# ztaylor797/APMBackend

Measured on AMD Instinct MI355X. Metric: log-lines/sec z-scored (whole node), higher is better.
Workload: dtype fp64

## Files before the change

### apmbackend_amd/csrc/kernels/devjoin.hip

```cpp
#include "kernel_api.h"

#include <rocprim/rocprim.hpp>

#include <chrono>
#include <climits>
#include <cstdlib>
#include <cstddef>
#include <cstring>
#include <vector>

#include "devjoin_api.h"
#include "devjoin_dev.h"
#include "devscan.h"
#include "prim.h"
#include "textout.h"

namespace apm {
using namespace dj;

namespace {

constexpr int TB = 256;

__device__ __forceinline__ uint32_t grid_n(uint32_t n) { return (n + TB - 1) / TB; }
// ... 2254 lines not shown

int apm_dj_take_marks(double* t, const char** names, int cap) {
  const int k = std::min(g_mark_k, cap);
  for (int i = 0; i < k; ++i) { t[i] = g_mark_t[i]; names[i] = g_mark_n[i]; }
  g_mark_k = 0;
  return k;
}

static int dj_sort_keys(PrimScratch& sc, const uint64_t* key, uint64_t* key_sorted, const uint32_t* val,
                        uint32_t* val_sorted, size_t n, hipStream_t s) {
  return prim_sort_pairs(sc, key, key_sorted, val, val_sorted, n, s);
}
static int dj_scan_counts(PrimScratch& sc, const uint32_t* cnt, uint32_t* pos, size_t n, hipStream_t s) {
  return prim_exclusive_scan(sc, cnt, pos, 0u, n, rocprim::plus<uint32_t>(), s);
}
static int dj_scan_lens(PrimScratch& sc, const U4* lens, U4* offs, size_t n, hipStream_t s) {
  return prim_exclusive_scan(sc, lens, offs, U4{0, 0, 0, 0}, n, U4Plus(), s);
}
static int dj_scan_bucket_max(PrimScratch& sc, const int64_t* bucket, int64_t* bmax, size_t n, hipStream_t s) {
  return prim_inclusive_scan(sc, bucket, bmax, n, rocprim::maximum<int64_t>(), s);
}

size_t apm_dj_tmp_bytes(uint32_t max_ev, uint32_t max_out) {
  PrimScratch q;
  const size_t n = std::max<size_t>(max_ev, 1) + 1;
  dj_sort_keys(q, nullptr, nullptr, nullptr, nullptr, n, 0);
  dj_scan_counts(q, nullptr, nullptr, n, 0);
  dj_scan_lens(q, nullptr, nullptr, (size_t)max_out + 1, 0);
  dj_scan_bucket_max(q, nullptr, nullptr, (size_t)max_out + 1, 0);
  return q.need + 4096;
}

int apm_dj_select_host(DJArgs* a, const uint32_t* d_n_ev, uint32_t max_ev, hipStream_t s) {
  HIP_OK(hipMemsetAsync(a->n_host, 0, sizeof(SelCount), s));
  if (max_ev == 0) return 0;
  uint32_t* list = reinterpret_cast<uint32_t*>(a->sel_pos);
  uint32_t* list_n = list + max_ev;
  HIP_OK(hipMemsetAsync(list_n, 0, 8, s));
  const dim3 grid((max_ev + TB - 1) / TB);
  hipLaunchKernelGGL(k_host_flags, grid, dim3(TB), 0, s, a->ev, d_n_ev, a->bytes, a->host_flag, a->sel_val, a->aud,
                     a->n_host, max_ev, list, list_n);
  dj_check(s, "k_host_flags");
  hipLaunchKernelGGL(k_host_flags_bytes, grid, dim3(TB), 0, s, a->ev, a->bytes, a->chunk_file, a->file_fkey,
                     a->host_flag, a->sel_val, a->aud, max_ev, list, list_n);
  dj_check(s, "k_host_flags_bytes");
  uint64_t* total = a->sel_pos + (max_ev + DS_TILE - 1) / DS_TILE + 1;
  if (ds_scan_apply<uint64_t>(SelValF{a->sel_val},
                              SelScatterG{a->ev, a->host_flag, total, a->host_ev, a->host_ev_idx, a->mh_idx,
                                          a->walk_idx, a->n_host},
                              d_n_ev, max_ev, a->sel_pos, total, s) != 0)
    return -1;
  dj_check(s, "k_ds_scan (host selection)");
  return 0;
}

static int apm_dj_audit(DJArgs* a, bool filled, hipStream_t s) {
  if (a->n_files && !filled) HIP_OK(hipMemsetAsync(a->gout.carry, 0, (size_t)a->n_files * sizeof(AudCarry), s));
  const uint32_t N = a->gin.n_autr + a->n_mh;
  if (N) {
    hipLaunchKernelGGL(k_aud_keys, dim3((N + TB - 1) / TB), dim3(TB), 0, s, *a);
    dj_check(s, "k_aud_keys");
    PrimScratch sc(a->tmp, a->tmp_bytes);
    if (dj_sort_keys(sc, a->aud_key, a->aud_key_sorted, a->aud_ord, a->aud_ord_sorted, N, s) != 0) return -1;
    dj_check(s, "rocprim_radix_sort_pairs");
    hipLaunchKernelGGL(k_aud_autr, dim3((N + TB - 1) / TB), dim3(TB), 0, s, *a);
    dj_check(s, "k_aud_autr");
  }
  if (a->n_walk || a->gin.n_txt) {
    if (a->n_files && !filled) HIP_OK(hipMemsetAsync(a->file_first_chunk, 0xff, (size_t)a->n_files * 4, s));
    const uint32_t lanes = std::max(a->n_chunks + 1, a->n_walk + 1);
    hipLaunchKernelGGL(k_aud_chunks, dim3((lanes + TB - 1) / TB), dim3(TB), 0, s, *a);
// ... 319 lines not shown
```

### apmbackend_amd/csrc/kernels/devjoin_api.h

```cpp
#pragma once
#include <vector>
#include <hip/hip_runtime.h>
#include <stdint.h>

#include "../apm_types.h"
#include "devjoin_types.h"

namespace apm {

constexpr int SOAP_SEGS = 16;
constexpr uint32_t DJ_OVF_CAP = 1u << 16;

enum : uint32_t {
  DJ_WRITE_OK = 0,
  DJ_WRITE_TXT = 1,
  DJ_WRITE_TOO_BIG = 2,
  DJ_WRITE_RING_FULL = 3,
};

__host__ __device__ inline uint64_t ring_place(uint64_t head, uint64_t bytes, uint64_t cap) {
  return ((head & (cap - 1)) + bytes > cap) ? (head + cap - 1) & ~(cap - 1) : head;
}

struct DJOverflow {
  uint32_t ev, sub;
  uint32_t pad[14];
  TxDev t;
};

struct AudGen {
  AudCarry* carry;
  AutrEnt* autr;
  AudItem* items;
  char* txt;
  uint32_t n_autr, n_items, n_txt;
  uint32_t cap_autr, cap_items, cap_txt;
};

struct SelCount {
  uint32_t host;
  uint32_t mh;
  uint32_t walk;
  uint32_t aud_bytes;
};

struct DJArgs {
  const Event* ev;
  uint32_t n_ev;
  const uint8_t* bytes;
  const uint32_t* chunk_file;
  const uint8_t* chunk_kind;
  uint32_t n_chunks;
  const int32_t* chunk_next;
  const uint8_t* chunk_first;
  const int32_t* file_server;
  const uint64_t* file_skey;
  const uint64_t* file_fkey;
  const HostOp* hops;
  uint32_t n_hops;
  const uint8_t* hbuf;
  double now;
  uint64_t batch_no;
  double rec_ttl, acct_ttl, need_ttl;
  uint8_t* host_flag;
  uint64_t* sel_val;
  uint64_t* sel_pos;
  Event* host_ev;
  uint32_t* host_ev_idx;
  uint32_t* mh_idx;
  uint32_t* walk_idx;
  SelCount* n_host;
  uint32_t n_mh, n_walk;
  uint32_t n_files;
  AudF* aud;
  AudGen gin, gout;
  uint64_t* aud_key;
  uint64_t* aud_key_sorted;
// ... 144 lines not shown
```

### apmbackend_amd/csrc/kernels/kernel_api.h

```cpp
#pragma once
#include <hip/hip_runtime.h>
#include <stdint.h>

#include "../apm_types.h"
#include "common.h"

namespace apm {

struct StatsState {
  int32_t* counts;
  int32_t* cells;
  int32_t* spill_n;
  int32_t* spill_series;
  int32_t* spill_val;
  uint8_t* active;
  int32_t cap;
  int32_t spill_cap;
  int32_t S;
  int32_t nslot = NSLOT_MIN;
  unsigned long long* spill_drop = nullptr;
  int32_t* nan_until = nullptr;
  int32_t* ord_list = nullptr;
  int32_t* ord_n = nullptr;
  uint32_t* ord_done = nullptr;
// ... 41 lines not shown
  int32_t rs_lo, rs_n, rs_parts;
  int32_t rs_mfma;
  double* rs_part;
  int32_t* rs_cnt;
};

constexpr int ROLLUP_ACC = 6;
constexpr int ROLLUP_OUT = 15;
constexpr int CTX_FIELDS = 18;
struct RollupArgs {
  const WinStat* win;
  const int32_t* series_server;
  const ZOut* z[MAX_LAGS];
  int32_t n_lags;
  int32_t n_series;
  int32_t n_servers;
  int64_t edge_ts;
  double tpm_div;
  const double* ctx;
  unsigned long long* acc;
  double* out;
};

struct CopySeg {
  void* dst;
  const void* src;
  size_t bytes;
};
struct CopySegs {
  CopySeg seg[8];
  int32_t n = 0;
  void add(void* d, const void* s, size_t b) {
    if (b) seg[n++] = CopySeg{d, s, b};
  }
};

struct ExportArgs {
  static constexpr int kMax = 8;
  void* src[kMax];
  void* dst[kMax];
  uint64_t reset_val[kMax];
  uint8_t bytes[kMax];
  uint8_t reset[kMax];
  int32_t n;
  void add(void* s, void* d, int nb, bool rst = false, uint64_t rv = 0) {
    src[n] = s; dst[n] = d; bytes[n] = (uint8_t)nb; reset[n] = rst ? 1 : 0; reset_val[n] = rv; ++n;
  }
};

struct FormatArgs {
  const int32_t* perm;
  const WinStat* win;
  const ZOut* z[MAX_LAGS];
  const int4* series_names;
  const char* names;
  int64_t edge_ts;
  int32_t n;
  int32_t n_lags;
  int32_t lag_order[MAX_LAGS];
  int32_t lag_value[MAX_LAGS];
  int32_t want_st, want_fs;
  int32_t fs_copy;
  uint32_t stage_hint;
  int32_t ts_copy_len;
  char ts_copy[32];
  int32_t ts_wire_len;
// ... 222 lines not shown
```

### apmbackend_amd/csrc/kernels/stats.hip

```cpp
#include "kernel_api.h"

#include "prim.h"
#include "spill.h"
#include "winsort.h"

#include <algorithm>
#include <cstdlib>

namespace apm {

constexpr int WS_WAVES = 4;
constexpr int WS_TILE = 1024;
constexpr int BIG_TILE = 16384;

__global__ void k_bucket_append(const TxRec* __restrict__ tx, uint32_t lo, uint32_t hi, StatsState st,
                                int64_t min_live_bucket) {
  const uint32_t i = lo + blockIdx.x * blockDim.x + threadIdx.x;
  if (i >= hi) return;
  const TxRec r = tx[i];
  if (r.series < 0 || r.series >= st.S) return;
  st.active[r.series] = 1;
  const int64_t b = r.end_ms / 10000;
  if (b < min_live_bucket) return;
  if (st.nan_until && b <= (int64_t)st.nan_until[r.series]) {
// ... 709 lines not shown
  for (; i < n; i += stride) dst[i] = src[i];
  if (t0 < tail) tdst[t0] = tsrc[t0];
}

}

__global__ void k_ck_lens(const int32_t* __restrict__ counts, const int32_t* __restrict__ slots, int k, int32_t n,
                          int32_t S, int32_t cap, uint32_t* __restrict__ lens) {
  const uint64_t t = (uint64_t)blockIdx.x * blockDim.x + threadIdx.x;
  const uint64_t N = (uint64_t)k * n;
  if (t > N) return;
  if (t == N) { lens[N] = 0; return; }
  const int i = (int)(t / (uint64_t)n), s = (int)(t % (uint64_t)n);
  const int32_t c = counts[(size_t)slots[i] * S + s];
  lens[t] = (uint32_t)(c < cap ? (c > 0 ? c : 0) : cap);
}

__global__ void k_ck_pack(const int32_t* __restrict__ cells, const int32_t* __restrict__ slots, int k, int32_t n,
                          int32_t S, int32_t cap, const uint32_t* __restrict__ lens, const uint32_t* __restrict__ offs,
                          int32_t* __restrict__ packed) {
  const uint64_t t = (uint64_t)blockIdx.x * blockDim.x + threadIdx.x;
  if (t >= (uint64_t)k * n) return;
  const int i = (int)(t / (uint64_t)n), s = (int)(t % (uint64_t)n);
  const int32_t* src = cells + ((size_t)slots[i] * S + s) * cap;
  int32_t* dst = packed + offs[t];
  for (uint32_t j = 0; j < lens[t]; ++j) dst[j] = src[j];
}

__global__ void k_copy_segs(apm::CopySegs c) {
  const apm::CopySeg& g = c.seg[blockIdx.y];
  if (blockIdx.y >= (unsigned)c.n) return;
  const size_t stride = (size_t)gridDim.x * blockDim.x;
  const size_t t = (size_t)blockIdx.x * blockDim.x + threadIdx.x;
  const uintptr_t al = (uintptr_t)g.dst | (uintptr_t)g.src;
  if ((al & 15) == 0) {
    const size_t n16 = g.bytes / 16;
    for (size_t i = t; i < n16; i += stride) reinterpret_cast<uint4*>(g.dst)[i] = reinterpret_cast<const uint4*>(g.src)[i];
    for (size_t i = n16 * 16 + t; i < g.bytes; i += stride) ((uint8_t*)g.dst)[i] = ((const uint8_t*)g.src)[i];
  } else if ((al & 3) == 0) {
    const size_t n4 = g.bytes / 4;
    for (size_t i = t; i < n4; i += stride) reinterpret_cast<uint32_t*>(g.dst)[i] = reinterpret_cast<const uint32_t*>(g.src)[i];
    for (size_t i = n4 * 4 + t; i < g.bytes; i += stride) ((uint8_t*)g.dst)[i] = ((const uint8_t*)g.src)[i];
  } else {
    for (size_t i = t; i < g.bytes; i += stride) ((uint8_t*)g.dst)[i] = ((const uint8_t*)g.src)[i];
  }
}

struct F64x8 {
  double v[8];
};
__global__ void k_set_f64(double* __restrict__ dst, F64x8 v, int n) {
  if ((int)threadIdx.x < n) dst[threadIdx.x] = v.v[threadIdx.x];
}

extern "C" {

using namespace apm;

void apm_copy(void* dst, const void* src, size_t bytes, hipStream_t stream) {
  apm_copy_capped(dst, src, bytes, 1024, stream);
}

void apm_copy_capped(void* dst, const void* src, size_t bytes, uint32_t max_blocks, hipStream_t stream) {
  if (bytes == 0) return;
  const uintptr_t a = (uintptr_t)dst | (uintptr_t)src;
  auto launch = [&](auto* d, const auto* s, size_t w) {
// ... 147 lines not shown
```

### apmbackend_amd/csrc/runtime/devjoin.cpp

```cpp
#include "devjoin.h"

#include <algorithm>
#include <chrono>
#include <climits>
#include <cstddef>
#include <cstdlib>
#include <cstring>
#include <stdexcept>

#include "../kernels/common.h"
#include "binio.h"
#include "d2h.h"
#include "../kernels/devjoin_dev.h"
#include "../kernels/kernel_api.h"
#include "join_util.h"
#include "jsutil.h"

namespace apm {

using namespace jstr;

namespace {
double clock_ms() {
  return std::chrono::duration<double, std::milli>(std::chrono::steady_clock::now().time_since_epoch()).count();
// ... 6 lines not shown
  op.line = e.line;
  op.server = server;
  op.op = JOP_NONE;
  return op;
}

uint64_t pow2_at_least(uint64_t v) {
  uint64_t p = 1;
  while (p < v) p <<= 1;
  return p;
}
}

DeviceJoin::DeviceJoin(const DevJoinConfig& cfg, Dictionary* dict, const std::vector<FileInfo>* files,
                       const std::vector<std::string>* servers)
    : cfg_(cfg), dict_(dict), files_(files), servers_(servers) {
  cfg_.ring_bytes = pow2_at_least(std::max<uint64_t>(cfg_.ring_bytes, 1ull << 24));
  cfg_.arena_cap = (uint32_t)pow2_at_least(std::max<uint32_t>(cfg_.arena_cap, 1024));
  HIP_OK(hipSetDevice(cfg_.device));
  {
    int lo = 0, hi = 0;
    HIP_OK(hipDeviceGetStreamPriorityRange(&lo, &hi));
    const char* pe = std::getenv("APM_JOIN_PRIO");
    HIP_OK(hipStreamCreateWithPriority(&stream_, hipStreamNonBlocking, pe && pe[0] == '0' ? lo : hi));
    res_.adopt(stream_);
  }
  const uint32_t E = std::max<uint32_t>(cfg_.max_events, 1024);
  out_cap_ = 2 * E + (1u << 16);
  for (int k = 0; k < 2; ++k) {
    Slot& s = sl_[k];
    s.d_bytes = (uint8_t*)res_.dmalloc_on(stream_, cfg_.max_batch_bytes + 256);
    s.d_events = (Event*)res_.dmalloc_on(stream_, (size_t)E * sizeof(Event));
    s.host_flag = (uint8_t*)res_.dmalloc_on(stream_, E + 64);
    s.d_host_ev = (Event*)res_.dmalloc_on(stream_, (size_t)E * sizeof(Event));
    s.d_host_idx = (uint32_t*)res_.dmalloc_on(stream_, (size_t)E * 4);
    s.d_mh_idx = (uint32_t*)res_.dmalloc_on(stream_, (size_t)E * 4);
    s.d_walk_idx = (uint32_t*)res_.dmalloc_on(stream_, (size_t)E * 4);
    s.d_aud = (AudF*)res_.dmalloc_on(stream_, (size_t)E * sizeof(AudF));
    s.d_n_host = (SelCount*)res_.dmalloc_on(stream_, 64);
    res_.pin(s.h_host_ev, (size_t)E * sizeof(Event));
    res_.pin(s.h_host_idx, (size_t)E * 4);
    res_.pin(s.h_n_host, 64);
    std::memset(s.h_n_host, 0, 64);
    s.d_chunk_next = (int32_t*)res_.dmalloc_on(stream_, ((size_t)cfg_.max_chunks + 2) * 4);
    s.d_chunk_first = (uint8_t*)res_.dmalloc_on(stream_, (size_t)cfg_.max_chunks + 2);
    res_.pin(s.h_chunk_next, ((size_t)cfg_.max_chunks + 2) * 4);
    res_.pin(s.h_chunk_first, (size_t)cfg_.max_chunks + 2);
    s.d_tx = (TxRec*)res_.dmalloc_on(stream_, (size_t)out_cap_ * sizeof(TxRec));
    s.d_tx_raw = (int32_t*)res_.dmalloc_on(stream_, (size_t)out_cap_ * 4);
    s.d_tx_gid = (int64_t*)res_.dmalloc_on(stream_, (size_t)out_cap_ * 8);
    s.free_ev = res_.new_event();
  }
  table_cap_ = 1u << cfg_.table_bits;
  init_table_cap_ = table_cap_;
  init_arena_cap_ = cfg_.arena_cap;
  d_table_ = (KeyState*)res_.dmalloc_on(stream_, (size_t)table_cap_ * sizeof(KeyState));
  d_reg_ = (RegSlot*)res_.dmalloc_on(stream_, ((size_t)1 << cfg_.reg_bits) * sizeof(RegSlot));
  miss_cap_ = E;
  d_miss_ = (RegMiss*)res_.dmalloc_on(stream_, (size_t)miss_cap_ * sizeof(RegMiss));
  res_.pin(h_miss_, (size_t)miss_cap_ * sizeof(RegMiss));
  d_arena_ = (NeedEnt*)res_.dmalloc_on(stream_, (size_t)cfg_.arena_cap * sizeof(NeedEnt));
  d_exp_lo_ = (uint64_t*)res_.dmalloc_on(stream_, 8 * 4096);
  d_exp_hi_ = (uint64_t*)res_.dmalloc_on(stream_, 8 * 4096);
  res_.pin(h_exp_, 2 * 8 * 4096);
  soap_cap_ = 1u << 16;
  d_soap_ = (SoapState*)res_.dmalloc_on(stream_, (size_t)soap_cap_ * sizeof(SoapState));
  if (E >= (1u << 21)) throw std::runtime_error("device join: gpu.maxLinesPerBatch must be below 2^21");
  d_sel_val_ = (uint64_t*)res_.dmalloc_on(stream_, ((size_t)E + 64) * 8);
  d_sel_pos_ = (uint64_t*)res_.dmalloc_on(stream_, ((size_t)E + 64) * 8);
  d_walk_lo_ = (uint32_t*)res_.dmalloc_on(stream_, ((size_t)cfg_.max_chunks + 2) * 4);
  d_file_first_ = (int32_t*)res_.dmalloc_on(stream_, (size_t)soap_cap_ * 4);
  for (AudGen& g : aud_gen_) {
    g.carry = (AudCarry*)res_.dmalloc_on(stream_, (size_t)soap_cap_ * sizeof(AudCarry));
    aud_reserve(g, 4096, 16384, 1u << 20);
  }
  d_file_server_ = (int32_t*)res_.dmalloc_on(stream_, (size_t)soap_cap_ * 4);
// ... 77 lines not shown
DeviceJoin::~DeviceJoin() {
  hipStreamSynchronize(stream_);
  res_.release_all();
}

void DeviceJoin::sync_file_keys() {
  const size_t n = files_->size();
  if (n <= h_file_fkey_.size()) return;
  if (n > soap_cap_) throw std::runtime_error("device join: too many files");
  const size_t lo = h_file_fkey_.size();
  if (lo == 0) HIP_OK(hipStreamSynchronize(stream_));
  for (size_t i = lo; i < n; ++i) {
    const FileInfo& f = (*files_)[i];
    const std::string& srv = (*servers_)[f.server];
    h_file_skey_.push_back(dj::server_key_of(srv.data(), srv.size()));
    h_file_fkey_.push_back(dj::file_key_of(f.path.data(), f.path.size()));
  }
  HIP_OK(hipMemcpy(d_file_skey_ + lo, h_file_skey_.data() + lo, (n - lo) * 8, hipMemcpyHostToDevice));
  HIP_OK(hipMemcpy(d_file_fkey_ + lo, h_file_fkey_.data() + lo, (n - lo) * 8, hipMemcpyHostToDevice));
}

void DeviceJoin::select_host(int k, const uint32_t* d_n_ev, uint32_t max_ev, hipStream_t ps) {
  Slot& s = sl_[k];
  sync_file_keys();
  DJArgs a{};
  a.ev = s.d_events;
  a.bytes = s.d_bytes;
  a.host_flag = s.host_flag;
  a.chunk_file = s.d_chunk_file;
  a.file_fkey = d_file_fkey_;
  a.aud = s.d_aud;
  a.sel_val = d_sel_val_;
  a.sel_pos = d_sel_pos_;
  a.host_ev = s.d_host_ev;
  a.host_ev_idx = s.d_host_idx;
  a.mh_idx = s.d_mh_idx;
  a.walk_idx = s.d_walk_idx;
  a.n_host = s.d_n_host;
  a.tmp = d_sel_tmp_;
  a.tmp_bytes = sel_tmp_bytes_;
  if (apm_dj_select_host(&a, d_n_ev, std::min<uint32_t>(max_ev, cfg_.max_events), ps) != 0)
    throw std::runtime_error("device join: scan scratch too small");
  HIP_OK(hipMemcpyAsync(s.h_n_host, s.d_n_host, sizeof(SelCount), hipMemcpyDeviceToHost, ps));
  s.spec = std::min<uint32_t>(cfg_.max_events, last_host_ + last_host_ / 4 + 256);
  HIP_OK(hipMemcpyAsync(s.h_host_ev, s.d_host_ev, (size_t)s.spec * sizeof(Event), hipMemcpyDeviceToHost, ps));
  HIP_OK(hipMemcpyAsync(s.h_host_idx, s.d_host_idx, (size_t)s.spec * 4, hipMemcpyDeviceToHost, ps));
}

void DeviceJoin::set_chunks(int k, const std::vector<int32_t>& chunk_file, const uint32_t* d_chunk_file,
                            const uint8_t* d_chunk_kind, hipStream_t ps) {
  Slot& s = sl_[k];
  const uint32_t n = (uint32_t)chunk_file.size();
  std::unordered_map<int32_t, int32_t> last;
  for (uint32_t c = 0; c < n; ++c) {
    s.h_chunk_next[c] = -1;
    auto it = last.find(chunk_file[c]);
    if (it == last.end()) {
      s.h_chunk_first[c] = 1;
    } else {
      s.h_chunk_first[c] = 0;
      s.h_chunk_next[it->second] = (int32_t)c;
    }
    last[chunk_file[c]] = (int32_t)c;
  }
  if (n) {
    HIP_OK(hipMemcpyAsync(s.d_chunk_next, s.h_chunk_next, (size_t)n * 4, hipMemcpyHostToDevice, ps));
    HIP_OK(hipMemcpyAsync(s.d_chunk_first, s.h_chunk_first, n, hipMemcpyHostToDevice, ps));
  }
  s.d_chunk_file = d_chunk_file;
  s.d_chunk_kind = d_chunk_kind;
  s.n_chunks = n;
  s.chunk_file = chunk_file;
}

void DeviceJoin::finish_select(int k, hipStream_t ps) {
  Slot& s = sl_[k];
  const uint32_t n = s.h_n_host->host;
  if (n > s.spec) {
    HIP_OK(hipMemcpyAsync(s.h_host_ev + s.spec, s.d_host_ev + s.spec, (size_t)(n - s.spec) * sizeof(Event),
                          hipMemcpyDeviceToHost, ps));
    HIP_OK(hipMemcpyAsync(s.h_host_idx + s.spec, s.d_host_idx + s.spec, (size_t)(n - s.spec) * 4,
                          hipMemcpyDeviceToHost, ps));
    HIP_OK(hipStreamSynchronize(ps));
  }
  last_host_ = n;
}

void DeviceJoin::host_prepass(int k, const uint8_t* hb, uint32_t n_host, const ParallelFor& parallel,
                              std::vector<HostOp>& hops_out, std::string& hbuf_out) {
  Slot& s = sl_[k];
  hops_out.clear();
  hbuf_out.clear();
  std::unordered_map<int32_t, int> task_of;
  int nt = 0;
  int32_t last_file = -1;
  int last_t = -1;
  for (uint32_t i = 0; i < n_host; ++i) {
    const int32_t file = s.chunk_file[s.h_host_ev[i].chunk];
    if (file == last_file) {
      tasks_[last_t].idx.push_back(i);
      continue;
    }
    auto it = task_of.find(file);
    int t;
    if (it == task_of.end()) {
      t = nt++;
      task_of.emplace(file, t);
      if ((int)tasks_.size() < nt) tasks_.emplace_back();
      PrepassTask& T = tasks_[t];
      T.file = file;
      T.idx.clear(); T.hops.clear(); T.hbuf.clear();
      T.audit_errors = T.invalid_acct = T.pm_host = 0;
    } else {
      t = it->second;
    }
    last_file = file;
    last_t = t;
    tasks_[t].idx.push_back(i);
// ... 483 lines not shown
    HIP_OK(hipEventSynchronize(live_ev_));
    keys_live_ = *h_live_;
    live_pending_ = false;
  }
  if ((keys_live_ + keys_since_rebuild_ + n_ev) * 2 > table_cap_) {
    if (table_rebuilds_ > 0 && async_rebuild_fits(n_ev)) {
      rebuild_table_async(now);
      return ensure_rest(n_ev, bytes);
    }
    rebuild_table(now, table_cap_);
    uint64_t cap = table_cap_;
    while ((keys_live_ + n_ev) * 2 > cap) cap *= 2;
    if (cap >= (1ull << 31)) throw std::runtime_error("device join: key table beyond 2^31 slots");
    if (cap != table_cap_) rebuild_table(now, (uint32_t)cap);
  }
  ensure_rest(n_ev, bytes);
}

void DeviceJoin::ensure_rest(uint32_t n_ev, uint64_t bytes) {
  {
    const uint64_t low = regions_.empty() ? arena_head_ : regions_.front().lo;
    const uint64_t used = arena_head_ - low;
    uint64_t cap = cfg_.arena_cap;
    while (cap - used < n_ev) cap *= 2;
    if (cap >= (1ull << 31)) throw std::runtime_error("device join: need arena beyond 2^31 entries");
    if (cap != cfg_.arena_cap) grow_arena((uint32_t)cap, low);
  }
  const uint64_t need = 2ull * n_ev + bytes / LBLK_N + 64;
  if (pool_avail(false) < need && pool_avail(true) < need) grow_pool(need);
}

void DeviceJoin::prepass_ahead(int k, const uint8_t* hb, const ParallelFor& parallel) {
  if (ahead_k_ >= 0) throw std::runtime_error("device join: a pre-pass is already ahead");
  host_prepass(k, hb, sl_[k].h_n_host->host, parallel, hops_ahead_, hbuf_ahead_);
  ahead_k_ = k;
}

void DeviceJoin::run(int k, const uint8_t* hb, uint32_t n_ev, uint64_t n_bytes, double now, uint64_t batch_no,
                     bool want_tx, bool want_db, DevJoinBatch& out, const ParallelFor& parallel,
                     const std::function<void()>* meanwhile) {
  Slot& s = sl_[k];
  hipStream_t st = stream_;
  if (n_ev > cfg_.max_events) throw std::runtime_error("device join: more events than maxLinesPerBatch");
  events_ += n_ev;
  phase_t[0] = clock_ms();
  if (ahead_k_ == k) {
    std::swap(hops_, hops_ahead_);
    std::swap(hbuf_, hbuf_ahead_);
    ahead_k_ = -1;
  } else {
    if (ahead_k_ >= 0) throw std::runtime_error("device join: pre-pass ahead for another slot");
    host_prepass(k, hb, s.h_n_host->host, parallel, hops_, hbuf_);
  }
  phase_t[1] = clock_ms();
  spans.clear();
  double sp = phase_t[1];
  auto span = [&](const char* name) { const double t = clock_ms(); spans.push_back({name, {sp, t}}); sp = t; };
  res_.reserve(h_hops_, hops_.size(), hops_.size() * 2 + 65536, true);
  res_.reserve(h_hbuf_, hbuf_.size(), hbuf_.size() * 2 + (4 << 20), true);
  span("u.hostgrow");
  if (hops_.size() > d_hops_cap_) {
    d_hops_cap_ = hops_.size() * 2 + 65536;
    d_hops_ = (HostOp*)res_.dmalloc_raw(d_hops_cap_ * sizeof(HostOp));
  }
  if (hbuf_.size() > d_hbuf_cap_) {
    d_hbuf_cap_ = hbuf_.size() * 2 + (4 << 20);
    d_hbuf_ = (uint8_t*)res_.dmalloc_raw(d_hbuf_cap_);
  }
  span("u.devgrow");
  if (!hops_.empty()) {
    std::memcpy(h_hops_, hops_.data(), hops_.size() * sizeof(HostOp));
    span("u.hops.memcpy");
    apm_copy(d_hops_, h_hops_.d, hops_.size() * sizeof(HostOp), st);
    span("u.hops.h2d");
  }
  if (!hbuf_.empty()) {
    std::memcpy(h_hbuf_, hbuf_.data(), hbuf_.size());
    span("u.hbuf.memcpy");
    apm_copy(d_hbuf_, h_hbuf_.d, hbuf_.size(), st);
    span("u.hbuf.h2d");
  }
  sync_file_keys();
  if (files_->size() > files_uploaded_) {
    if (files_->size() > soap_cap_) throw std::runtime_error("device join: too many files");
    std::vector<int32_t> fs(files_->size() - files_uploaded_);
// ... 704 lines not shown
```

### apmbackend_amd/csrc/runtime/devjoin.h

```cpp
#pragma once
#include <hip/hip_runtime.h>

#include <atomic>
#include <cstdint>
#include <deque>
#include <functional>
#include <mutex>
#include <string>
#include <unordered_map>
#include <vector>

#include "../apm_types.h"
#include "../kernels/devjoin_api.h"
#include "hipres.h"
#include "join.h"

namespace apm {

struct DevJoinConfig {
  uint32_t max_events = 1u << 20;
  uint64_t max_batch_bytes = 64ull << 20;
  uint32_t max_chunks = 4096;
  int table_bits = 21;
  int reg_bits = 20;
  uint32_t max_raw = 1u << 20;
  uint32_t arena_cap = 1u << 20;
  uint32_t pool_blocks = 0;
  uint64_t ring_bytes = 4ull << 30;
  double record_ttl_ms = 120000, acct_ttl_ms = 120000, need_ttl_ms = 30000;
  TzTable tz{};
  int device = 0;
};

struct DevJoinBatch {
  int slot = 0;
  uint32_t n_out = 0, n_stats = 0, n_db = 0, n_dropped = 0;
  std::vector<std::pair<uint32_t, int64_t>> cands;
  std::vector<std::pair<uint32_t, int32_t>> unresolved;
  std::string text_tx, text_db;
  uint64_t ring_base = 0;
  int64_t max_bucket = INT64_MIN;
  TxRec* d_tx = nullptr;
  int32_t* d_raw = nullptr;
  int64_t* d_gid = nullptr;
};

class DeviceJoin {
 public:
  DeviceJoin(const DevJoinConfig& cfg, Dictionary* dict, const std::vector<FileInfo>* files,
             const std::vector<std::string>* servers);
  ~DeviceJoin();

  uint8_t* d_bytes(int k) { return sl_[k].d_bytes; }
  uint8_t* d_stage() {
    if (!d_stage_bytes_) {
      d_stage_bytes_ = (uint8_t*)res_.dmalloc_on(stream_, cfg_.max_batch_bytes + 256);
      HIP_OK(hipStreamSynchronize(stream_));
    }
    return d_stage_bytes_;
  }
  void swap_stage(int k) { std::swap(sl_[k].d_bytes, d_stage_bytes_); }
  Event* d_events(int k) { return sl_[k].d_events; }
  void select_host(int k, const uint32_t* d_n_ev, uint32_t max_ev, hipStream_t ps);
  void set_chunks(int k, const std::vector<int32_t>& chunk_file, const uint32_t* d_chunk_file,
                  const uint8_t* d_chunk_kind, hipStream_t ps);
  void finish_select(int k, hipStream_t ps);
  using ParallelFor = std::function<void(int, const std::function<void(int)>&)>;
  void run(int k, const uint8_t* host_bytes, uint32_t n_ev, uint64_t n_bytes, double now, uint64_t batch_no, bool want_tx,
           bool want_db, DevJoinBatch& out, const ParallelFor& parallel = nullptr,
           const std::function<void()>* meanwhile = nullptr);
  void prepass_ahead(int k, const uint8_t* host_bytes, const ParallelFor& parallel);
  void release_slot(int k, hipStream_t stats_stream);

  int32_t raw_server(int32_t raw) const { return raw_info_[raw].server; }
  int32_t raw_service(int32_t raw) const { return raw_info_[raw].norm_id; }
  int32_t n_raw() const { return n_raw_.load(std::memory_order_acquire); }
  int32_t* d_raw_series() { return d_raw_series_; }

  char* ring() { return d_ring_; }
  uint64_t ring_cap() const { return cfg_.ring_bytes; }
  void set_ring_low(uint64_t low);
  uint64_t ring_head() const { return ring_head_.load(std::memory_order_acquire); }
  uint64_t ring_low() const { return ring_low_.load(std::memory_order_acquire); }
  uint64_t keys_live() const { return keys_live_ + keys_since_rebuild_; }
  uint64_t need_live() const { return arena_head_ - (regions_.empty() ? arena_head_ : regions_.front().lo); }
  uint64_t ring_reserve(uint64_t bytes);
  void reset_ring(uint64_t head);

  JoinCounters counters() const;
  std::vector<uint64_t> cache_stats(double now, bool sync = true);

  void save(class BinWriter& w);
  void load(class BinReader& r);
  static constexpr int kPhases = 8;
  double phase_t[kPhases + 1] = {0};
  std::vector<std::pair<const char*, std::pair<double, double>>> spans;
  std::vector<std::pair<const char*, std::pair<double, double>>> save_spans;
  const JoinCounts& last_counts() const { return *h_counts_; }
  size_t device_bytes() const { return res_.device_bytes(); }
  size_t trim(double now);

 private:
  struct Slot {
    uint8_t* d_bytes = nullptr;
    Event* d_events = nullptr;
    uint8_t* host_flag = nullptr;
    Event* d_host_ev = nullptr;
    uint32_t* d_host_idx = nullptr;
    uint32_t* d_mh_idx = nullptr;
    uint32_t* d_walk_idx = nullptr;
    AudF* d_aud = nullptr;
    SelCount* d_n_host = nullptr;
    Event* h_host_ev = nullptr;
    uint32_t* h_host_idx = nullptr;
    SelCount* h_n_host = nullptr;
    uint32_t spec = 0;
    int32_t* d_chunk_next = nullptr;
    uint8_t* d_chunk_first = nullptr;
    int32_t* h_chunk_next = nullptr;
    uint8_t* h_chunk_first = nullptr;
    const uint32_t* d_chunk_file = nullptr;
    const uint8_t* d_chunk_kind = nullptr;
    uint32_t n_chunks = 0;
    std::vector<int32_t> chunk_file;
    TxRec* d_tx = nullptr;
    int32_t* d_tx_raw = nullptr;
    int64_t* d_tx_gid = nullptr;
    hipEvent_t free_ev = nullptr;
    bool used = false;
  } sl_[2];

  struct RawInfo { int32_t server; int32_t norm_id; uint64_t svc; };

  struct PrepassTask {
    int32_t file = -1;
    std::vector<uint32_t> idx;
    std::vector<HostOp> hops;
    std::string hbuf;
    uint64_t audit_errors = 0, invalid_acct = 0, pm_host = 0;
    uint32_t put(std::string_view s) { const uint32_t o = (uint32_t)hbuf.size(); hbuf.append(s.data(), s.size()); return o; }
  };
  void host_prepass(int k, const uint8_t* host_bytes, uint32_t n_host, const ParallelFor& parallel,
                    std::vector<HostOp>& hops, std::string& hbuf);
  void host_event(PrepassTask& t, const Event& e, uint32_t ev, const uint8_t* host_bytes);
  void on_app(PrepassTask& t, const Event& e, uint32_t ev, std::string_view line);
  void save_tables(class BinWriter& w);
  void aud_reserve(AudGen& g, uint32_t autr, uint32_t items, uint64_t txt);
  int32_t intern_name(const std::string& s);
  void register_misses(const uint8_t* host_bytes, uint32_t n_miss, hipStream_t s);
  void ensure_capacity(uint32_t n_ev, uint64_t bytes, double now);
  void rebuild_table(double now, uint32_t new_cap);
  void rebuild_table_async(double now);
  bool async_rebuild_fits(uint64_t n_ev) const {
    return (keys_live_ + keys_since_rebuild_ + n_ev) * 8 <= (uint64_t)table_cap_ * 5;
  }
  void ensure_rest(uint32_t n_ev, uint64_t bytes);
  void rebuild_inplace(double now);
  void idle_upkeep(double now, uint32_t n_next);
  void grow_arena(uint32_t new_cap, uint64_t lo);
  void grow_pool(uint64_t need_free);
  uint64_t pool_avail(bool exact);
  void ensure_tmp();

  DevJoinConfig cfg_;
  uint32_t init_table_cap_ = 0, init_arena_cap_ = 0;
  Dictionary* dict_;
  const std::vector<FileInfo>* files_;
  const std::vector<std::string>* servers_;
  hipStream_t stream_ = nullptr;
  HipRes res_;
  uint8_t* d_stage_bytes_ = nullptr;

  std::vector<HostOp> hops_;
  std::string hbuf_;
  std::vector<HostOp> hops_ahead_;
  std::string hbuf_ahead_;
  int ahead_k_ = -1;
  PinnedBuf<HostOp> h_hops_;
  PinnedBuf<uint8_t> h_hbuf_;
  HostOp* d_hops_ = nullptr;
  uint8_t* d_hbuf_ = nullptr;
  size_t d_hops_cap_ = 0, d_hbuf_cap_ = 0;
  std::vector<PrepassTask> tasks_;
  uint32_t last_host_ = 0;
  void* d_sel_tmp_ = nullptr;
  size_t sel_tmp_bytes_ = 0;
  uint64_t audit_errors_ = 0, host_pm_ = 0, host_invalid_acct_ = 0, host_events_ = 0, events_ = 0, tx_ = 0, tx_db_ = 0;

  DJArgs a_{};
  DJFormatArgs f_{};
  KeyState* d_table_ = nullptr;
  uint64_t* d_keys_ = nullptr;
  uint32_t keys_cap_ = 0;
  bool keys_stale_ = true;
  void sync_keys();
  unsigned long long* d_cstats_ = nullptr;
  unsigned long long* h_cstats_ = nullptr;
  unsigned long long cstats_last_[5] = {0, 0, 0, 0, 0};
  uint32_t cstats_cap_ = 0, cstats_last_cap_ = 0;
  hipEvent_t cstats_ev_ = nullptr;
  bool cstats_pending_ = false, cstats_have_ = false;
  KeyState* d_table_spare_ = nullptr;
  uint32_t table_cap_ = 0;
  uint64_t keys_since_rebuild_ = 0, keys_live_ = 0;
  bool live_pending_ = false;
  hipEvent_t live_ev_ = nullptr;
  uint32_t* d_rb_scratch_ = nullptr;
  size_t rb_scratch_bytes_ = 0;
  uint8_t* d_pool_ = nullptr;
  uint32_t* d_pool_ring_ = nullptr;
  uint32_t pool_n_ = 0;
  unsigned long long* h_live_ = nullptr;
  uint64_t table_grows_ = 0, arena_grows_ = 0, pool_grows_ = 0, table_rebuilds_ = 0, trims_ = 0;
  RegSlot* d_reg_ = nullptr;
  RegMiss* d_miss_ = nullptr;
  RegMiss* h_miss_ = nullptr;
  uint32_t miss_cap_ = 0;
// ... 92 lines not shown
```

### apmbackend_amd/csrc/runtime/engine.cpp

```cpp
#include <cstdlib>
#include "engine.h"

#include <pthread.h>
#include <sched.h>

#include <cctype>
#include <fstream>

#include <rocprofiler-sdk-roctx/roctx.h>

#include <unistd.h>

#include <cerrno>
#include <cstring>

#include <algorithm>
#include <exception>
#include <chrono>
#include <cmath>
#include <cstring>
#include <queue>
#include <stdexcept>

#include "../kernels/devjoin_api.h"
// ... 773 lines not shown
      const Chunk& c = chunks_in[order[k]];
      const uint64_t len = c.end - c.begin;
      if (len > 0 && src[c.end - 1] != '\n') throw std::runtime_error("chunk must end with a newline");
      std::memcpy(ps.h_bytes + off, src + c.begin, len);
      ps.h_chunk_begin[k] = (uint32_t)off;
      ps.h_chunk_kind[k] = files_[c.file].kind;
      ps.h_chunk_file[k] = (uint32_t)c.file;
      ps.chunk_file[k] = c.file;
      off += len;
    }
    std::memset(ps.h_bytes + off, 0, 64);
  }
  const uint32_t n_chunks = (uint32_t)order.size();
  ps.h_chunk_begin[n_chunks] = (uint32_t)off;
  ps.n_bytes = off;
  ps.src = host_bytes;
  ps.src_n = n_bytes;
  metrics_.bytes += off;
  ++metrics_.batches;

  const int k = (int)(&ps - pslot_);
  bool staged = false;
  if (dev() && canonical && in_stage_src_ == host_bytes && in_stage_n_ == n_bytes && in_stage_ev_) {
    HIP_OK(hipStreamWaitEvent(parse_stream_, in_stage_ev_, 0));
    dj_->swap_stage(k);
    staged = true;
    ++metrics_.staged_batches;
  }
  in_stage_src_ = nullptr;
  in_stage_n_ = 0;
  uint8_t* dbytes = dev() ? dj_->d_bytes(k) : d_bytes_;
  Event* devents = dev() ? dj_->d_events(k) : d_events_;
  if (!staged) HIP_OK(hipMemcpyAsync(dbytes, ps.hb, off, hipMemcpyHostToDevice, parse_stream_));
  h2d(d_chunk_begin_[k], ps.h_chunk_begin, (n_chunks + 1) * 4, parse_stream_);
  h2d(d_chunk_kind_[k], ps.h_chunk_kind, n_chunks + 1, parse_stream_);
  h2d(d_chunk_file_[k], ps.h_chunk_file, (n_chunks + 1) * 4, parse_stream_);
  if (apm_parse_batch(dbytes, off, d_chunk_begin_[k], d_chunk_kind_[k], d_chunk_file_[k], n_chunks, d_parse_ws_,
                      cfg_.max_lines, devents, d_counts_, d_counts_ + 1, d_watermark_, d_file_open_, &cfg_.tz,
                      parse_stream_) != 0)
    throw std::runtime_error("parse workspace too small");
  if (dev()) {
    dj_->set_chunks(k, ps.chunk_file, d_chunk_file_[k], d_chunk_kind_[k], parse_stream_);
    dj_->select_host(k, d_counts_, cfg_.max_lines, parse_stream_);
  }
  d2h(ps.h_counts, d_counts_, 8, parse_stream_);
  d2h(ps.h_watermark, d_watermark_, 8, parse_stream_);
  ps.spec_copied = 0;
  if (speculative && !dev() && spec_events_) {
    ps.spec_copied = std::min<uint32_t>(spec_events_, cfg_.max_lines);
    HIP_OK(hipMemcpyAsync(ps.h_events, d_events_, (size_t)ps.spec_copied * sizeof(Event), hipMemcpyDeviceToHost,
                          parse_stream_));
  }
  ps.pending = true;
  metrics_.t_parse_ms += now_ms() - t0;
}

void Engine::stage_batch(const uint8_t* host_bytes, uint64_t n_bytes) {
  if (!dev() || !host_bytes || n_bytes == 0 || n_bytes > cfg_.max_batch_bytes) return;
  const double t0 = now_ms();
  if (!in_stage_stream_) {
    HIP_OK(hipStreamCreateWithFlags(&in_stage_stream_, hipStreamNonBlocking));
    res_.adopt(in_stage_stream_);
    in_stage_ev_ = res_.new_event();
  }
  HIP_OK(hipMemcpyAsync(dj_->d_stage(), host_bytes, n_bytes, hipMemcpyHostToDevice, in_stage_stream_));
  HIP_OK(hipEventRecord(in_stage_ev_, in_stage_stream_));
  in_stage_src_ = host_bytes;
  in_stage_n_ = n_bytes;
  trace_event("stage H2D (launch)", t0, now_ms(), 0);
}

void Engine::finish_parse(ParseSlot& ps) {
  const double t0 = now_ms();
  HIP_OK(hipStreamSynchronize(parse_stream_));
  ps.n_events = ps.h_counts[0];
  ps.n_lines = ps.h_counts[1];
  if (ps.n_lines > cfg_.max_lines) throw std::runtime_error("batch has more lines than max_lines");
  metrics_.lines += ps.n_lines;
  metrics_.events += ps.n_events;
  if (dev()) {
    dj_->finish_select((int)(&ps - pslot_), parse_stream_);
  } else if (ps.n_events > ps.spec_copied) {
    const uint32_t lo = ps.spec_copied;
    HIP_OK(hipMemcpyAsync(ps.h_events + lo, d_events_ + lo, (size_t)(ps.n_events - lo) * sizeof(Event),
                          hipMemcpyDeviceToHost, parse_stream_));
    HIP_OK(hipStreamSynchronize(parse_stream_));
  }
  ps.spec_copied = 0;
  spec_events_ = ps.n_events + ps.n_events / 4 + 1024;
  ps.pending = false;
  last_slot_ = (int)(&ps - pslot_);
  metrics_.t_parse_ms += now_ms() - t0;
}

static void merge_shard_outputs(const std::vector<std::vector<TxOut>>& outs, bool multi, std::vector<TxOut>& txs) {
  txs.clear();
  const int ns = (int)outs.size();
  size_t total = 0;
  std::vector<size_t> split(ns, 0);
  for (int k = 0; k < ns; ++k) {
    auto& v = outs[k];
    total += v.size();
    size_t p = 0;
    while (p < v.size() && !(v[p].seq >> 63)) ++p;
    split[k] = p;
  }
  txs.reserve(total);
  using Item = std::pair<uint64_t, std::pair<int, size_t>>;
  std::priority_queue<Item, std::vector<Item>, std::greater<Item>> pq;
  for (int k = 0; k < ns; ++k)
    if (split[k] > 0) pq.push({outs[k][0].seq, {k, 0}});
  while (!pq.empty()) {
    auto it = pq.top();
    pq.pop();
    auto& v = outs[it.second.first];
// ... 2785 lines not shown
```

Before: 308.4 million.

## Batch small parse-stage copies into one kernel and write host selection to mapped memory

Replaces several small hipMemcpyAsync/hipMemsetAsync calls around parsing with single copy-segment kernel launches that read and write host-mapped pinned buffers through device aliases, and adds zero-fill support to that kernel. The host-selected events and indices are now written directly into mapped host memory by the scatter kernel, removing the speculative D2H copies and the follow-up synchronising catch-up copy. This is meant to cut per-batch API and launch overhead and a possible extra stream sync. In exchange, kernels write over PCIe/fabric into host memory, which may be slower per byte than DMA.

```diff
diff --git a/apmbackend_amd/csrc/kernels/devjoin.hip b/apmbackend_amd/csrc/kernels/devjoin.hip
--- a/apmbackend_amd/csrc/kernels/devjoin.hip
+++ b/apmbackend_amd/csrc/kernels/devjoin.hip
@@ -2310,11 +2310,9 @@
 }
 
 int apm_dj_select_host(DJArgs* a, const uint32_t* d_n_ev, uint32_t max_ev, hipStream_t s) {
-  HIP_OK(hipMemsetAsync(a->n_host, 0, sizeof(SelCount), s));
   if (max_ev == 0) return 0;
   uint32_t* list = reinterpret_cast<uint32_t*>(a->sel_pos);
-  uint32_t* list_n = list + max_ev;
-  HIP_OK(hipMemsetAsync(list_n, 0, 8, s));
+  uint32_t* list_n = dj_select_list_n(a->sel_pos, max_ev);
   const dim3 grid((max_ev + TB - 1) / TB);
   hipLaunchKernelGGL(k_host_flags, grid, dim3(TB), 0, s, a->ev, d_n_ev, a->bytes, a->host_flag, a->sel_val, a->aud,
                      a->n_host, max_ev, list, list_n);
diff --git a/apmbackend_amd/csrc/kernels/devjoin_api.h b/apmbackend_amd/csrc/kernels/devjoin_api.h
--- a/apmbackend_amd/csrc/kernels/devjoin_api.h
+++ b/apmbackend_amd/csrc/kernels/devjoin_api.h
@@ -43,6 +43,10 @@
   uint32_t walk;
   uint32_t aud_bytes;
 };
+
+inline uint32_t* dj_select_list_n(uint64_t* sel_pos, uint32_t max_ev) {
+  return reinterpret_cast<uint32_t*>(sel_pos) + max_ev;
+}
 
 struct DJArgs {
   const Event* ev;
diff --git a/apmbackend_amd/csrc/kernels/kernel_api.h b/apmbackend_amd/csrc/kernels/kernel_api.h
--- a/apmbackend_amd/csrc/kernels/kernel_api.h
+++ b/apmbackend_amd/csrc/kernels/kernel_api.h
@@ -97,6 +97,9 @@
   int32_t n = 0;
   void add(void* d, const void* s, size_t b) {
     if (b) seg[n++] = CopySeg{d, s, b};
+  }
+  void zero(void* d, size_t b) {
+    if (b) seg[n++] = CopySeg{d, nullptr, b};
   }
 };
 
diff --git a/apmbackend_amd/csrc/kernels/stats.hip b/apmbackend_amd/csrc/kernels/stats.hip
--- a/apmbackend_amd/csrc/kernels/stats.hip
+++ b/apmbackend_amd/csrc/kernels/stats.hip
@@ -765,6 +765,10 @@
   if (blockIdx.y >= (unsigned)c.n) return;
   const size_t stride = (size_t)gridDim.x * blockDim.x;
   const size_t t = (size_t)blockIdx.x * blockDim.x + threadIdx.x;
+  if (!g.src) {
+    for (size_t i = t; i < g.bytes; i += stride) ((uint8_t*)g.dst)[i] = 0;
+    return;
+  }
   const uintptr_t al = (uintptr_t)g.dst | (uintptr_t)g.src;
   if ((al & 15) == 0) {
     const size_t n16 = g.bytes / 16;
diff --git a/apmbackend_amd/csrc/runtime/devjoin.cpp b/apmbackend_amd/csrc/runtime/devjoin.cpp
--- a/apmbackend_amd/csrc/runtime/devjoin.cpp
+++ b/apmbackend_amd/csrc/runtime/devjoin.cpp
@@ -62,8 +62,6 @@
     s.d_bytes = (uint8_t*)res_.dmalloc_on(stream_, cfg_.max_batch_bytes + 256);
     s.d_events = (Event*)res_.dmalloc_on(stream_, (size_t)E * sizeof(Event));
     s.host_flag = (uint8_t*)res_.dmalloc_on(stream_, E + 64);
-    s.d_host_ev = (Event*)res_.dmalloc_on(stream_, (size_t)E * sizeof(Event));
-    s.d_host_idx = (uint32_t*)res_.dmalloc_on(stream_, (size_t)E * 4);
     s.d_mh_idx = (uint32_t*)res_.dmalloc_on(stream_, (size_t)E * 4);
     s.d_walk_idx = (uint32_t*)res_.dmalloc_on(stream_, (size_t)E * 4);
     s.d_aud = (AudF*)res_.dmalloc_on(stream_, (size_t)E * sizeof(AudF));
@@ -71,7 +69,7 @@
     res_.pin(s.h_host_ev, (size_t)E * sizeof(Event));
     res_.pin(s.h_host_idx, (size_t)E * 4);
     res_.pin(s.h_n_host, 64);
-    std::memset(s.h_n_host, 0, 64);
+    std::memset(s.h_n_host.h, 0, 64);
     s.d_chunk_next = (int32_t*)res_.dmalloc_on(stream_, ((size_t)cfg_.max_chunks + 2) * 4);
     s.d_chunk_first = (uint8_t*)res_.dmalloc_on(stream_, (size_t)cfg_.max_chunks + 2);
     res_.pin(s.h_chunk_next, ((size_t)cfg_.max_chunks + 2) * 4);
@@ -215,8 +213,8 @@
   a.aud = s.d_aud;
   a.sel_val = d_sel_val_;
   a.sel_pos = d_sel_pos_;
-  a.host_ev = s.d_host_ev;
-  a.host_ev_idx = s.d_host_idx;
+  a.host_ev = s.h_host_ev.d;
+  a.host_ev_idx = s.h_host_idx.d;
   a.mh_idx = s.d_mh_idx;
   a.walk_idx = s.d_walk_idx;
   a.n_host = s.d_n_host;
@@ -224,14 +222,24 @@
   a.tmp_bytes = sel_tmp_bytes_;
   if (apm_dj_select_host(&a, d_n_ev, std::min<uint32_t>(max_ev, cfg_.max_events), ps) != 0)
     throw std::runtime_error("device join: scan scratch too small");
-  HIP_OK(hipMemcpyAsync(s.h_n_host, s.d_n_host, sizeof(SelCount), hipMemcpyDeviceToHost, ps));
-  s.spec = std::min<uint32_t>(cfg_.max_events, last_host_ + last_host_ / 4 + 256);
-  HIP_OK(hipMemcpyAsync(s.h_host_ev, s.d_host_ev, (size_t)s.spec * sizeof(Event), hipMemcpyDeviceToHost, ps));
-  HIP_OK(hipMemcpyAsync(s.h_host_idx, s.d_host_idx, (size_t)s.spec * 4, hipMemcpyDeviceToHost, ps));
+}
+
+void DeviceJoin::export_select(int k, CopySegs& cs) {
+  Slot& s = sl_[k];
+  cs.add(s.h_n_host.d, s.d_n_host, sizeof(SelCount));
+}
+
+void DeviceJoin::chunk_upload(int k, uint32_t max_ev, CopySegs& cs) {
+  Slot& s = sl_[k];
+  cs.add(s.d_chunk_next, s.h_chunk_next.d, (size_t)s.n_chunks * 4);
+  cs.add(s.d_chunk_first, s.h_chunk_first.d, s.n_chunks);
+  max_ev = std::min<uint32_t>(max_ev, cfg_.max_events);
+  cs.zero(s.d_n_host, sizeof(SelCount));
+  if (max_ev) cs.zero(dj_select_list_n(d_sel_pos_, max_ev), 8);
 }
 
 void DeviceJoin::set_chunks(int k, const std::vector<int32_t>& chunk_file, const uint32_t* d_chunk_file,
-                            const uint8_t* d_chunk_kind, hipStream_t ps) {
+                            const uint8_t* d_chunk_kind) {
   Slot& s = sl_[k];
   const uint32_t n = (uint32_t)chunk_file.size();
   std::unordered_map<int32_t, int32_t> last;
@@ -246,27 +254,10 @@
     }
     last[chunk_file[c]] = (int32_t)c;
   }
-  if (n) {
-    HIP_OK(hipMemcpyAsync(s.d_chunk_next, s.h_chunk_next, (size_t)n * 4, hipMemcpyHostToDevice, ps));
-    HIP_OK(hipMemcpyAsync(s.d_chunk_first, s.h_chunk_first, n, hipMemcpyHostToDevice, ps));
-  }
   s.d_chunk_file = d_chunk_file;
   s.d_chunk_kind = d_chunk_kind;
   s.n_chunks = n;
   s.chunk_file = chunk_file;
-}
-
-void DeviceJoin::finish_select(int k, hipStream_t ps) {
-  Slot& s = sl_[k];
-  const uint32_t n = s.h_n_host->host;
-  if (n > s.spec) {
-    HIP_OK(hipMemcpyAsync(s.h_host_ev + s.spec, s.d_host_ev + s.spec, (size_t)(n - s.spec) * sizeof(Event),
-                          hipMemcpyDeviceToHost, ps));
-    HIP_OK(hipMemcpyAsync(s.h_host_idx + s.spec, s.d_host_idx + s.spec, (size_t)(n - s.spec) * 4,
-                          hipMemcpyDeviceToHost, ps));
-    HIP_OK(hipStreamSynchronize(ps));
-  }
-  last_host_ = n;
 }
 
 void DeviceJoin::host_prepass(int k, const uint8_t* hb, uint32_t n_host, const ParallelFor& parallel,
@@ -816,7 +807,7 @@
 
 void DeviceJoin::prepass_ahead(int k, const uint8_t* hb, const ParallelFor& parallel) {
   if (ahead_k_ >= 0) throw std::runtime_error("device join: a pre-pass is already ahead");
-  host_prepass(k, hb, sl_[k].h_n_host->host, parallel, hops_ahead_, hbuf_ahead_);
+  host_prepass(k, hb, sl_[k].h_n_host.h->host, parallel, hops_ahead_, hbuf_ahead_);
   ahead_k_ = k;
 }
 
@@ -834,7 +825,7 @@
     ahead_k_ = -1;
   } else {
     if (ahead_k_ >= 0) throw std::runtime_error("device join: pre-pass ahead for another slot");
-    host_prepass(k, hb, s.h_n_host->host, parallel, hops_, hbuf_);
+    host_prepass(k, hb, s.h_n_host.h->host, parallel, hops_, hbuf_);
   }
   phase_t[1] = clock_ms();
   spans.clear();
diff --git a/apmbackend_amd/csrc/runtime/devjoin.h b/apmbackend_amd/csrc/runtime/devjoin.h
--- a/apmbackend_amd/csrc/runtime/devjoin.h
+++ b/apmbackend_amd/csrc/runtime/devjoin.h
@@ -16,6 +16,8 @@
 #include "join.h"
 
 namespace apm {
+
+struct CopySegs;
 
 struct DevJoinConfig {
   uint32_t max_events = 1u << 20;
@@ -63,8 +65,9 @@
   Event* d_events(int k) { return sl_[k].d_events; }
   void select_host(int k, const uint32_t* d_n_ev, uint32_t max_ev, hipStream_t ps);
   void set_chunks(int k, const std::vector<int32_t>& chunk_file, const uint32_t* d_chunk_file,
-                  const uint8_t* d_chunk_kind, hipStream_t ps);
-  void finish_select(int k, hipStream_t ps);
+                  const uint8_t* d_chunk_kind);
+  void chunk_upload(int k, uint32_t max_ev, CopySegs& cs);
+  void export_select(int k, CopySegs& cs);
   using ParallelFor = std::function<void(int, const std::function<void(int)>&)>;
   void run(int k, const uint8_t* host_bytes, uint32_t n_ev, uint64_t n_bytes, double now, uint64_t batch_no, bool want_tx,
            bool want_db, DevJoinBatch& out, const ParallelFor& parallel = nullptr,
@@ -105,20 +108,17 @@
     uint8_t* d_bytes = nullptr;
     Event* d_events = nullptr;
     uint8_t* host_flag = nullptr;
-    Event* d_host_ev = nullptr;
-    uint32_t* d_host_idx = nullptr;
     uint32_t* d_mh_idx = nullptr;
     uint32_t* d_walk_idx = nullptr;
     AudF* d_aud = nullptr;
     SelCount* d_n_host = nullptr;
-    Event* h_host_ev = nullptr;
-    uint32_t* h_host_idx = nullptr;
-    SelCount* h_n_host = nullptr;
-    uint32_t spec = 0;
+    Mapped<Event> h_host_ev;
+    Mapped<uint32_t> h_host_idx;
+    Mapped<SelCount> h_n_host;
     int32_t* d_chunk_next = nullptr;
     uint8_t* d_chunk_first = nullptr;
-    int32_t* h_chunk_next = nullptr;
-    uint8_t* h_chunk_first = nullptr;
+    Mapped<int32_t> h_chunk_next;
+    Mapped<uint8_t> h_chunk_first;
     const uint32_t* d_chunk_file = nullptr;
     const uint8_t* d_chunk_kind = nullptr;
     uint32_t n_chunks = 0;
@@ -182,7 +182,6 @@
   uint8_t* d_hbuf_ = nullptr;
   size_t d_hops_cap_ = 0, d_hbuf_cap_ = 0;
   std::vector<PrepassTask> tasks_;
-  uint32_t last_host_ = 0;
   void* d_sel_tmp_ = nullptr;
   size_t sel_tmp_bytes_ = 0;
   uint64_t audit_errors_ = 0, host_pm_ = 0, host_invalid_acct_ = 0, host_events_ = 0, events_ = 0, tx_ = 0, tx_db_ = 0;
diff --git a/apmbackend_amd/csrc/runtime/engine.cpp b/apmbackend_amd/csrc/runtime/engine.cpp
--- a/apmbackend_amd/csrc/runtime/engine.cpp
+++ b/apmbackend_amd/csrc/runtime/engine.cpp
@@ -829,19 +829,29 @@
   uint8_t* dbytes = dev() ? dj_->d_bytes(k) : d_bytes_;
   Event* devents = dev() ? dj_->d_events(k) : d_events_;
   if (!staged) HIP_OK(hipMemcpyAsync(dbytes, ps.hb, off, hipMemcpyHostToDevice, parse_stream_));
-  h2d(d_chunk_begin_[k], ps.h_chunk_begin, (n_chunks + 1) * 4, parse_stream_);
-  h2d(d_chunk_kind_[k], ps.h_chunk_kind, n_chunks + 1, parse_stream_);
-  h2d(d_chunk_file_[k], ps.h_chunk_file, (n_chunks + 1) * 4, parse_stream_);
+  {
+    CopySegs up;
+    up.add(d_chunk_begin_[k], HipRes::device_alias(ps.h_chunk_begin), (size_t)(n_chunks + 1) * 4);
+    up.add(d_chunk_kind_[k], HipRes::device_alias(ps.h_chunk_kind), n_chunks + 1);
+    up.add(d_chunk_file_[k], HipRes::device_alias(ps.h_chunk_file), (size_t)(n_chunks + 1) * 4);
+    if (dev()) {
+      dj_->set_chunks(k, ps.chunk_file, d_chunk_file_[k], d_chunk_kind_[k]);
+      dj_->chunk_upload(k, cfg_.max_lines, up);
+    }
+    apm_copy_segs(&up, parse_stream_);
+  }
   if (apm_parse_batch(dbytes, off, d_chunk_begin_[k], d_chunk_kind_[k], d_chunk_file_[k], n_chunks, d_parse_ws_,
                       cfg_.max_lines, devents, d_counts_, d_counts_ + 1, d_watermark_, d_file_open_, &cfg_.tz,
                       parse_stream_) != 0)
     throw std::runtime_error("parse workspace too small");
-  if (dev()) {
-    dj_->set_chunks(k, ps.chunk_file, d_chunk_file_[k], d_chunk_kind_[k], parse_stream_);
-    dj_->select_host(k, d_counts_, cfg_.max_lines, parse_stream_);
-  }
-  d2h(ps.h_counts, d_counts_, 8, parse_stream_);
-  d2h(ps.h_watermark, d_watermark_, 8, parse_stream_);
+  if (dev()) dj_->select_host(k, d_counts_, cfg_.max_lines, parse_stream_);
+  {
+    CopySegs ex;
+    ex.add(HipRes::device_alias(ps.h_counts), d_counts_, 8);
+    ex.add(HipRes::device_alias(ps.h_watermark), d_watermark_, 8);
+    if (dev()) dj_->export_select(k, ex);
+    apm_copy_segs(&ex, parse_stream_);
+  }
   ps.spec_copied = 0;
   if (speculative && !dev() && spec_events_) {
     ps.spec_copied = std::min<uint32_t>(spec_events_, cfg_.max_lines);
@@ -875,9 +885,7 @@
   if (ps.n_lines > cfg_.max_lines) throw std::runtime_error("batch has more lines than max_lines");
   metrics_.lines += ps.n_lines;
   metrics_.events += ps.n_events;
-  if (dev()) {
-    dj_->finish_select((int)(&ps - pslot_), parse_stream_);
-  } else if (ps.n_events > ps.spec_copied) {
+  if (!dev() && ps.n_events > ps.spec_copied) {
     const uint32_t lo = ps.spec_copied;
     HIP_OK(hipMemcpyAsync(ps.h_events + lo, d_events_ + lo, (size_t)(ps.n_events - lo) * sizeof(Event),
                           hipMemcpyDeviceToHost, parse_stream_));
```

After: 322.0 million, median of 6. 4.4% higher.
